# ORNL/MultiDistTorch

Hardware: AMD Instinct MI355X
Metric: aggregate VAE samples/sec across K concurrent HPO trials (higher is better)
Workload: dtype bf16; 1 GPU; model=conv-VAE 28x28 (2 conv + 2 deconv, z=32), global_batch=128, per_trial_batch=128, image=28, parallelism=groups1x1, trials=1, backend=hip, graphs=True, timing_barrier=none, valid=True

## Files before the change

### csrc/kernels/conv_igemm.h

```cpp
#pragma once
#include <stdint.h>

namespace mdt {

struct ConvDesc {
  int N, H, W, C;
  int OH, OW, CO;
  int KH, KW, S, P;
};

struct FastDiv {
  uint32_t d, mul, shr;
};

inline FastDiv make_fastdiv(uint32_t d) {
  FastDiv f;
  f.d = d;
  f.shr = 0;
  while ((1u << f.shr) < d) ++f.shr;
  const uint64_t one = 1;
  f.mul = (uint32_t)(((one << 32) * ((one << f.shr) - d)) / d + 1);
  return f;
}

enum IgemmMode : int {
  kModeConv = 0,
  kModeTconv = 1,
};

struct FwdPlan {
  int cfg;
  int BM, BN;
  int classes;
  int M;
  int Ncols, K;
  int mtiles, ntiles, ktiles;
  int ksplit, kt_per_split;
  int colsum_rows;
  int thin;
  int direct;
};

struct WgradPlan {
  int cfg;
  int BM, BN;
  int M, K2;
  int cotiles, ktiles, mtiles;
  int nsplit, mt_per_split;
  int thin;
};

struct APro {
  const float* slab;
  const float* bias;
  void* out16;
  int ks, relu, cin;
  long long stride;
};

struct GradSeg {
  long long off, numel;
  const float* slab;
  int nsplit;
  int co, k, s, ci;
  long long toff;
};

struct GradUnit {
  int seg, start, count;
};

struct TrUnit {
  int seg, tap, co0, ci0;
};

constexpr int kJobArgBytes = 256;
struct JobBlob {
  int kind;
  int nblk;
  int aux[6];
  alignas(16) unsigned char args[kJobArgBytes];
};

enum JobKindBase : int {
  kJobIgemm = 1000,
  kJobWgrad = 2000,
  kJobWgradThin = 2050,
  kJobThinWgM = 2100,
  kJobWgradAdam = 2200,
  kJobThinConv = 3000,
  kJobThinTconv = 4000,
  kJobColsum = 5000,
  kJobLoss = 5001,
  kJobCombine = 5002,
  kJobFinalize = 5003,
  kJobWtrans = 5004,
  kJobLossStep = 5005,
  kJobComm = 5006,
  kJobDconv = 6000,
};

constexpr int kMaxMultiJobs = 8;

}
```

### csrc/kernels/conv_igemm.hip

```cpp
#include <algorithm>

#include "conv_igemm_dev.h"
#include "conv_direct.h"
#include "conv_dwgrad.h"
#include "conv_thin_wg.h"

namespace mdt {

__global__ void __launch_bounds__(256) splitk_combine_k(CombineArgs c) {
  __shared__ float red[256];
  splitk_combine_body(c, red, blockIdx.x);
}

__global__ void __launch_bounds__(256) colsum_k(ColsumArgs c) { colsum_body(c, blockIdx.x); }

}

using namespace mdt;

namespace {
inline int cdiv(long long a, long long b) { return (int)((a + b - 1) / b); }
}

namespace mdt {
using namespace mdt::tiles;

struct DcInfo {
  int RB, NBB, MT, NB;
};
template <class CF>
constexpr DcInfo dc_info() { return DcInfo{CF::RB, CF::NBB, CF::MT, CF::NB}; }
static const DcInfo kDcInfo[] = {dc_info<DcS1>(), dc_info<DcS2>(), dc_info<DcT2>(),
                                  dc_info<DcT3>(), dc_info<DcS3>(), dc_info<DcT1>()};

static bool direct_small() {
  static const bool on = [] {
    const char* e = getenv("MDT_DCONV_SMALL");
    return !(e && e[0] == '0');
  }();
  return on;
}

int direct_cfg(int mode, const ConvDesc& d, bool fwd) {
  static const bool on = [] {
    const char* e = getenv("MDT_CONV_DIRECT");
    return !(e && e[0] == '0');
  }();
  static const bool bwd = [] {
    const char* e = getenv("MDT_DCONV_BWD");
    return !(e && e[0] == '0');
  }();
  if (!on || d.KH != 4 || d.KW != 4 || d.S != 2 || d.P != 1) return -1;
  if (!fwd && !bwd) return -1;
  if (d.H != d.W || d.OH != d.OW || d.H != 2 * d.OH) return -1;
  if (mode == kModeConv) {
    if (d.C == 32 && d.H == 64 && d.CO == 64) return 0;
    if (d.C == 64 && d.H == 32 && d.CO == 128) return 1;
    if (d.C == 128 && d.H == 16 && d.CO == 256 && fwd && direct_small()) return 4;
  } else {
    if (d.CO == 128 && d.OH == 16 && d.C == 64) return 2;
    if (d.CO == 64 && d.OH == 32 && d.C == 32) return 3;
    if (d.CO == 256 && d.OH == 8 && d.C == 128 && fwd && direct_small()) return 5;
  }
  return -1;
}

bool plan_fwd(int mode, const ConvDesc& d, bool allow_split, FwdPlan* p, bool allow_direct, bool fwd) {
  FwdPlan q{};
  const int dc = allow_direct ? direct_cfg(mode, d, fwd) : -1;
  if (dc >= 0) {
    const DcInfo& di = kDcInfo[dc];
    q.direct = dc + 1;
    q.classes = mode == kModeConv ? 1 : 4;
    q.M = mode == kModeConv ? d.N * d.OH * d.OW : d.N * d.OH * d.OW;
    q.Ncols = mode == kModeConv ? d.CO : d.C;
    q.K = mode == kModeConv ? 16 * d.C : 4 * d.CO;
    q.BM = di.MT; q.BN = di.NB;
    q.mtiles = d.N * di.RB; q.ntiles = di.NBB; q.ktiles = q.K / 64;
    q.ksplit = 1; q.kt_per_split = q.ktiles;
    q.colsum_rows = d.N * di.RB;
    q.cfg = 100 + dc;
    *p = q;
    return true;
  }
  if (mode == kModeConv) {
    q.classes = 1;
    q.M = d.N * d.OH * d.OW;
    q.Ncols = d.CO;
    q.K = d.KH * d.KW * d.C;
    q.thin = (d.C % 8) != 0;
  } else {
    if (d.KH % d.S || d.KW % d.S || d.H % d.S || d.W % d.S || d.CO % 8) return false;
    q.classes = d.S * d.S;
    q.M = d.N * (d.H / d.S) * (d.W / d.S);
    q.Ncols = d.C;
    q.K = (d.KH / d.S) * (d.KW / d.S) * d.CO;
    q.thin = 0;
  }
  if (q.K % 8 || q.M <= 0) return false;
  q.BN = q.Ncols >= 128 ? 128 : q.Ncols > 32 ? 64 : q.Ncols > 16 ? 32 : 16;
  if (q.thin) q.BN = 32;
  static const int bn_split_below = [] {
    const char* e = getenv("MDT_CONV_BN_SPLIT_BELOW");
    return e ? atoi(e) : 512;
  }();
  static const int bn_split_min_kt = [] {
    const char* e = getenv("MDT_CONV_BN_SPLIT_MIN_KT");
    return e ? atoi(e) : 16;
  }();
  static const int bn_split_tiny = [] {
    const char* e = getenv("MDT_CONV_BN_SPLIT_TINY");
    return e ? atoi(e) : 512;
  }();
  auto grid64 = [&] { return (long long)q.classes * cdiv(q.M, 64) * cdiv(q.Ncols, q.BN); };
  while (q.BN > 32 && !q.thin &&
         ((cdiv(q.K, 64) >= bn_split_min_kt && grid64() < bn_split_below) || grid64() < bn_split_tiny))
    q.BN /= 2;
  q.ntiles = cdiv(q.Ncols, q.BN);
  q.ktiles = cdiv(q.K, 64);
  static const int bm64_below = [] {
    const char* e = getenv("MDT_CONV_BM64_BELOW");
    return e ? atoi(e) : 1024;
  }();
  q.BM = 128;
  if ((long long)q.classes * cdiv(q.M, 128) * q.ntiles < bm64_below) q.BM = 64;
  q.mtiles = cdiv(q.M, q.BM);
  const long long blocks = (long long)q.classes * q.mtiles * q.ntiles;
  q.ksplit = 1;
  static const int min_kt = [] {
    const char* e = getenv("MDT_CONV_SPLIT_MIN_KT");
    return e ? atoi(e) : 8;
  }();
  static const int kt_per = [] {
    const char* e = getenv("MDT_CONV_SPLIT_KT_PER");
    const int v = e ? atoi(e) : 1;
    return v < 1 ? 1 : v;
  }();
  if (allow_split && q.classes == 1 && blocks < 256 && q.ktiles >= min_kt) {
    int ks = cdiv(512, blocks);
    if (ks > q.ktiles / kt_per) ks = q.ktiles / kt_per;
    if (ks < 1) ks = 1;
    q.ksplit = ks;
  }
  q.kt_per_split = cdiv(q.ktiles, q.ksplit);
  q.ksplit = cdiv(q.ktiles, q.kt_per_split);
  q.colsum_rows = q.classes * q.mtiles;
  const int bn_i = q.BN == 128 ? 0 : q.BN == 64 ? 1 : q.BN == 32 ? 2 : 3;
  q.cfg = (q.BM == 128 ? 0 : 4) + bn_i;
  *p = q;
  return true;
}

int dwgrad_cfg(const ConvDesc& d) {
  static const bool on = [] {
    const char* e = getenv("MDT_DWGRAD");
    return !(e && e[0] == '0');
  }();
  const char* e2 = getenv("MDT_DWGRAD_L2");
  const bool l2 = e2 && e2[0] == '1';
  if (!on || d.S != 2 || d.P != 1 || d.KH != 4 || d.KW != 4 || d.H != d.W || d.OH != d.OW || d.OH * 2 != d.H)
    return -1;
  if (d.H == DwL1::H && d.C == DwL1::C && d.CO == DwL1::CO) return 0;
  if (l2 && d.H == DwL2::H && d.C == DwL2::C && d.CO == DwL2::CO) return 1;
  return -1;
}

bool plan_wgrad(const ConvDesc& d, WgradPlan* p) {
  WgradPlan q{};
  if (d.CO % 8) return false;
  if (thin_wgrad_mfma_ok(d)) {
    q.cfg = 110;
    q.thin = true;
    q.M = d.N * d.OH * d.OW;
    q.K2 = d.KH * d.KW * d.C;
    q.BM = d.CO;
    q.BN = q.K2;
    q.cotiles = q.ktiles = 1;
    q.mtiles = d.N * d.OH / 4;
    q.nsplit = q.mtiles;
    q.mt_per_split = 1;
    *p = q;
    return true;
  }
  const int dw = dwgrad_cfg(d);
  if (dw >= 0) {
    q.cfg = 100 + dw;
    q.M = d.N * d.OH * d.OW;
    q.K2 = d.KH * d.KW * d.C;
    q.BM = d.CO;
    q.BN = q.K2;
    q.cotiles = q.ktiles = 1;
    q.mtiles = d.N;
    q.nsplit = d.N;
    q.mt_per_split = 1;
    *p = q;
    return true;
  }
  q.M = d.N * d.OH * d.OW;
  q.K2 = d.KH * d.KW * d.C;
  q.thin = (d.C % 8) != 0;
  q.BM = d.CO > 32 ? 64 : 32;
  q.BN = q.K2 > 32 ? 64 : q.K2 > 16 ? 32 : 16;
  if (q.thin && q.BN == 32) q.BN = 64;
  q.cotiles = cdiv(d.CO, q.BM);
  q.ktiles = cdiv(q.K2, q.BN);
  q.mtiles = cdiv(q.M, 64);
  const int tiles = q.cotiles * q.ktiles;
  static const int fixed_target = [] {
    const char* e = getenv("MDT_CONV_WG_TARGET");
    return e ? atoi(e) : 0;
  }();
  static const int thin_target = [] {
    const char* e = getenv("MDT_CONV_WG_TARGET_THIN");
    return e ? atoi(e) : 0;
  }();
  int target = q.thin && thin_target > 0 ? thin_target : fixed_target;
  if (target <= 0) {
    const long long work = (long long)q.mtiles * tiles;
    target = (int)std::min<long long>(640, std::max<long long>(160, work / 16));
  }
  int ns = cdiv(target, tiles);
  if (ns > q.mtiles / 2) ns = q.mtiles / 2;
  if (ns < 1) ns = 1;
  q.mt_per_split = cdiv(q.mtiles, ns);
  q.nsplit = cdiv(q.mtiles, q.mt_per_split);
  q.cfg = (q.BM == 64 ? 0 : 3) + (q.BN == 64 ? 0 : q.BN == 32 ? 1 : 2);
  *p = q;
  return true;
}

int build_igemm(int mode, const void* A, const void* B16, ConvDesc d, const float* bias, int relu, void* y16,
                float* y32, const void* omask, float* colsum, float* ws, IgArgs* pa, FwdPlan* pq, CombineArgs* pc,
                int* nc) {
  FwdPlan q;
  const bool can_split = ws != nullptr && omask == nullptr && colsum == nullptr;
  if (!plan_fwd(mode, d, can_split, &q, false)) return 1;
  IgArgs a{};
  a.d = d;
  a.A = A;
  a.B = reinterpret_cast<const __bf16*>(B16);
  a.relu = relu;
  a.M = q.M; a.Ncols = q.Ncols; a.K = q.K; a.mtiles = q.mtiles; a.ntiles = q.ntiles; a.ktiles = q.ktiles;
  a.kt_per_split = q.kt_per_split;
  if (mode == kModeConv) {
    a.f_pix = make_fastdiv(d.OH * d.OW); a.f_w = make_fastdiv(d.OW);
    a.f_ch = make_fastdiv(d.C); a.f_tw = make_fastdiv(d.KW);
  } else {
    a.f_pix = make_fastdiv((d.H / d.S) * (d.W / d.S)); a.f_w = make_fastdiv(d.W / d.S);
    a.f_ch = make_fastdiv(d.CO); a.f_tw = make_fastdiv(d.KW / d.S);
  }
  *nc = 0;
  if (q.ksplit > 1) {
    a.slab = ws;
    const long long MN = (long long)q.M * q.Ncols;
    int rp = 1;
    while (rp < 64 && rp * 4 < q.ksplit) rp *= 2;
    const int cnt = 256 / rp;
    *pc = CombineArgs{ws, q.ksplit, q.M, q.Ncols, cnt, bias, relu, y32, reinterpret_cast<__bf16*>(y16)};
    *nc = cdiv(MN, cnt);
  } else {
    a.y16 = reinterpret_cast<__bf16*>(y16); a.y32 = y32; a.bias = bias;
    a.omask = reinterpret_cast<const __bf16*>(omask); a.colsum = colsum;
  }
  *pa = a;
  *pq = q;
  return 0;
}

int build_wgrad(const void* G16, const void* X, ConvDesc d, float* out, WgArgs* pa, WgradPlan* pq) {
  WgradPlan q;
  if (!plan_wgrad(d, &q)) return 1;
  WgArgs a{};
  a.d = d;
  a.G = reinterpret_cast<const __bf16*>(G16);
  a.X = X;
  a.out = out;
  a.M = q.M; a.K2 = q.K2; a.cotiles = q.cotiles; a.ktiles = q.ktiles; a.mtiles = q.mtiles;
  a.mt_per_split = q.mt_per_split;
  a.f_pix = make_fastdiv(d.OH * d.OW); a.f_w = make_fastdiv(d.OW);
  a.f_c = make_fastdiv(d.C); a.f_kw = make_fastdiv(d.KW);
  *pa = a;
  *pq = q;
  return 0;
}

template <typename XT>
__global__ void __launch_bounds__(256) thin_wgrad_k(WgArgs a) {
  __shared__ __attribute__((aligned(16))) uint8_t lds[thin_wgrad_mfma_lds_bytes()];
  thin_wgrad_mfma_body<XT>(a, lds, blockIdx.x);
}

static unsigned long long* g_dc_stamps = nullptr;

template <class CF>
void launch_dc(const DcArgs& a, hipStream_t s) {
  hipLaunchKernelGGL((dconv_k<CF>), dim3(a.nimg * CF::RB * CF::NBB), dim3(CF::THREADS), 0, s, a);
}

int launch_direct(int cfg, const void* A, const void* B16, const ConvDesc& d, const float* bias, int relu, void* y16,
                  float* y32, const void* omask, float* colsum, hipStream_t s) {
  DcArgs a{};
  a.A = reinterpret_cast<const __bf16*>(A);
  a.B = reinterpret_cast<const __bf16*>(B16);
  a.y16 = reinterpret_cast<__bf16*>(y16);
  a.y32 = y32;
  a.bias = bias;
  a.omask = reinterpret_cast<const __bf16*>(omask);
  a.colsum = colsum;
  a.stamps = g_dc_stamps;
  a.relu = relu;
  a.nimg = d.N;
  switch (cfg) {
    case 0: launch_dc<DcS1>(a, s); break;
    case 1: launch_dc<DcS2>(a, s); break;
    case 2: launch_dc<DcT2>(a, s); break;
    case 3: launch_dc<DcT3>(a, s); break;
    case 4: launch_dc<DcS3>(a, s); break;
    case 5: launch_dc<DcT1>(a, s); break;
    default: return 2;
  }
  return (int)hipGetLastError();
}

int launch_splitk_combine(const CombineArgs& c, int nblk, hipStream_t s) {
  hipLaunchKernelGGL(splitk_combine_k, dim3(nblk), dim3(256), 0, s, c);
  return (int)hipGetLastError();
}

}

namespace {
using namespace mdt::tiles;

template <int MODE, typename AT, bool VEC, class TC, bool PRO = false>
void launch_fwd(const IgArgs& a, const FwdPlan& q, hipStream_t s) {
  dim3 grid(q.mtiles * q.ntiles, q.ksplit, q.classes);
  hipLaunchKernelGGL((igemm_fwd_k<MODE, AT, VEC, TC, PRO>), grid, dim3(256), 0, s, a);
}

template <int MODE, typename AT, bool VEC, bool PRO = false>
int dispatch_fwd_cfg(const IgArgs& a, const FwdPlan& q, hipStream_t s) {
  switch (q.cfg) {
    case 0: launch_fwd<MODE, AT, VEC, F0, PRO>(a, q, s); return 0;
    case 1: launch_fwd<MODE, AT, VEC, F1, PRO>(a, q, s); return 0;
    case 2: launch_fwd<MODE, AT, VEC, F2, PRO>(a, q, s); return 0;
    case 3: launch_fwd<MODE, AT, VEC, F3, PRO>(a, q, s); return 0;
    case 4: launch_fwd<MODE, AT, VEC, F4, PRO>(a, q, s); return 0;
    case 5: launch_fwd<MODE, AT, VEC, F5, PRO>(a, q, s); return 0;
    case 6: launch_fwd<MODE, AT, VEC, F6, PRO>(a, q, s); return 0;
    case 7: launch_fwd<MODE, AT, VEC, F7, PRO>(a, q, s); return 0;
  }
  return 2;
}

template <typename AT>
int dispatch_thin(const IgArgs& a, const FwdPlan& q, hipStream_t s) {
  if (q.cfg == 2) { launch_fwd<kModeConv, AT, false, F2>(a, q, s); return 0; }
  if (q.cfg == 6) { launch_fwd<kModeConv, AT, false, F6>(a, q, s); return 0; }
  return 2;
}

template <typename XT, bool VEC, class TC>
void launch_wg(const WgArgs& a, const WgradPlan& q, hipStream_t s) {
  dim3 grid(q.cotiles * q.ktiles * q.nsplit);
  hipLaunchKernelGGL((wgrad_k<XT, VEC, TC>), grid, dim3(256), 0, s, a);
}

}

extern "C" {

int mdt_igemm_plan(int mode, ConvDesc d, int allow_split, int* info, int fwd) {
  FwdPlan q;
  if (!plan_fwd(mode, d, allow_split != 0, &q, true, fwd != 0)) return 1;
  const int v[12] = {q.cfg, q.BM, q.BN, q.classes, q.M, q.Ncols, q.K, q.mtiles, q.ntiles, q.ktiles, q.ksplit,
                     q.colsum_rows};
  for (int i = 0; i < 12; ++i) info[i] = v[i];
  return 0;
}

int mdt_wgrad_plan(ConvDesc d, int* info) {
  WgradPlan q;
  if (!plan_wgrad(d, &q)) return 1;
  const int v[8] = {q.cfg, q.BM, q.BN, q.cotiles, q.ktiles, q.mtiles, q.nsplit, q.mt_per_split};
  for (int i = 0; i < 8; ++i) info[i] = v[i];
  return 0;
}

int mdt_igemm(int mode, const void* A, int a_is_f32, const void* B16, ConvDesc d, const float* bias, int relu,
              void* y16, float* y32, const void* omask, float* colsum, float* ws, int skip_combine, hipStream_t s,
              const APro* pro, int fwd) {
  IgArgs a;
  FwdPlan q;
  CombineArgs c;
  int nc = 0;
  const int dc = direct_cfg(mode, d, fwd != 0);
  if (dc >= 0) {
    if ((pro && pro->slab) || a_is_f32) return 5;
    return launch_direct(dc, A, B16, d, bias, relu, y16, y32, omask, colsum, s);
  }
  if (build_igemm(mode, A, B16, d, bias, relu, y16, y32, omask, colsum, ws, &a, &q, &c, &nc)) return 1;
  int rc;
  if (pro && pro->slab) {
    if (mode != kModeConv || q.thin || a_is_f32 || pro->cin % 8 || pro->ks < 1) return 4;
    a.pro = *pro;
    rc = dispatch_fwd_cfg<kModeConv, __bf16, true, true>(a, q, s);
  } else if (mode == kModeConv) {
    if (q.thin) rc = a_is_f32 ? dispatch_thin<float>(a, q, s) : dispatch_thin<__bf16>(a, q, s);
    else if (a_is_f32) rc = 3;
    else rc = dispatch_fwd_cfg<kModeConv, __bf16, true>(a, q, s);
  } else if (a_is_f32) {
    rc = 3;
  } else {
    rc = dispatch_fwd_cfg<kModeTconv, __bf16, true>(a, q, s);
  }
  if (rc) return rc;
  if (nc > 0 && !skip_combine) hipLaunchKernelGGL(splitk_combine_k, dim3(nc), dim3(256), 0, s, c);
  return (int)hipGetLastError();
}

int mdt_wgrad(const void* G16, const void* X, int x_is_f32, ConvDesc d, float* out, hipStream_t s) {
  WgArgs a;
  WgradPlan q;
  if (build_wgrad(G16, X, d, out, &a, &q)) return 1;
  if (q.cfg == 110) {
    if (x_is_f32) hipLaunchKernelGGL(thin_wgrad_k<float>, dim3(q.nsplit), dim3(256), 0, s, a);
    else hipLaunchKernelGGL(thin_wgrad_k<__bf16>, dim3(q.nsplit), dim3(256), 0, s, a);
    return (int)hipGetLastError();
  }
  if (q.cfg >= 100) {
    if (x_is_f32) return 3;
    const DwArgs da{reinterpret_cast<const __bf16*>(X), reinterpret_cast<const __bf16*>(G16), out, d.N, g_dc_stamps};
    if (q.cfg == 100) hipLaunchKernelGGL(dwgrad_k<DwL1>, dim3(d.N * 4), dim3(DwL1::THREADS), 0, s, da);
    else if (q.cfg == 101) hipLaunchKernelGGL(dwgrad_k<DwL2>, dim3(d.N * 4), dim3(DwL2::THREADS), 0, s, da);
    else return 2;
    return (int)hipGetLastError();
  }
  if (!q.thin) {
    if (x_is_f32) return 3;
    switch (q.cfg) {
      case 0: launch_wg<__bf16, true, W0>(a, q, s); break;
      case 1: launch_wg<__bf16, true, W1>(a, q, s); break;
      case 2: launch_wg<__bf16, true, W2>(a, q, s); break;
      case 3: launch_wg<__bf16, true, W3>(a, q, s); break;
      case 4: launch_wg<__bf16, true, W4>(a, q, s); break;
      case 5: launch_wg<__bf16, true, W5>(a, q, s); break;
      default: return 2;
    }
  } else {
    switch (q.cfg) {
      case 0: if (x_is_f32) launch_wg<float, false, W0>(a, q, s); else launch_wg<__bf16, false, W0>(a, q, s); break;
      case 2: if (x_is_f32) launch_wg<float, false, W2>(a, q, s); else launch_wg<__bf16, false, W2>(a, q, s); break;
      case 3: if (x_is_f32) launch_wg<float, false, W3>(a, q, s); else launch_wg<__bf16, false, W3>(a, q, s); break;
      case 5: if (x_is_f32) launch_wg<float, false, W5>(a, q, s); else launch_wg<__bf16, false, W5>(a, q, s); break;
      default: return 2;
    }
  }
  return (int)hipGetLastError();
}

void mdt_dconv_stamps(unsigned long long* p) { g_dc_stamps = p; }

int mdt_colsum(const void* G16, int M, int N, int rows_per, float* slab, hipStream_t s) {
  if (N % 8 || rows_per < 1) return 1;
  const int gx = cdiv(N / 8, 256);
  const ColsumArgs c{reinterpret_cast<const __bf16*>(G16), M, N, rows_per, gx, slab};
  hipLaunchKernelGGL(colsum_k, dim3(gx * cdiv(M, rows_per)), dim3(256), 0, s, c);
  return (int)hipGetLastError();
}

}
```

### csrc/kernels/conv_jobs.hip

```cpp
#include <string.h>

#include <algorithm>

#include "conv_direct.h"
#include "conv_dwgrad.h"
#include "conv_igemm_dev.h"
#include "comm_jobs.h"
#include "conv_small.h"
#include "conv_thin.h"
#include "conv_thin_wg.h"

namespace mdt {
using namespace tiles;

struct JobPack {
  JobBlob j[3];
  int start1, start2;
};

template <class T>
__device__ __forceinline__ const T& job_args(const JobBlob& j) {
  return *reinterpret_cast<const T*>(j.args);
}

struct JNone {
  static constexpr int ID = 0, LDS = 0;
  static __device__ __forceinline__ void run(const JobBlob&, uint8_t*, int) {}
};

template <int MODE, int CFG, class TC>
struct JIg {
  static constexpr int ID = kJobIgemm + MODE * 100 + CFG, LDS = igemm_lds_bytes<TC>();
  static __device__ __forceinline__ void run(const JobBlob& j, uint8_t* lds, int b) {
    const int ntb = j.aux[0], ks = j.aux[1];
    const int r = b / ntb, t = b - r * ntb;
    const int cls = r / ks, kz = r - cls * ks;
    igemm_body<MODE, __bf16, true, TC>(job_args<IgArgs>(j), lds, t, ntb, kz, cls);
  }
};

template <int CFG, class TC>
struct JWg {
  static constexpr int ID = kJobWgrad + CFG, LDS = wgrad_lds_bytes<TC>();
  static __device__ __forceinline__ void run(const JobBlob& j, uint8_t* lds, int b) {
    wgrad_body<__bf16, true, TC>(job_args<WgArgs>(j), lds, b, j.nblk);
  }
};

template <typename XT, int CFG, class TC>
struct JWgThin {
  static constexpr int ID = kJobWgradThin + (sizeof(XT) == 4 ? 20 : 0) + CFG, LDS = wgrad_lds_bytes<TC>();
  static __device__ __forceinline__ void run(const JobBlob& j, uint8_t* lds, int b) {
    wgrad_body<XT, false, TC>(job_args<WgArgs>(j), lds, b, j.nblk);
  }
};

template <typename XT>
struct JThinWg {
  static constexpr int ID = kJobThinWgM + (sizeof(XT) == 4 ? 1 : 0), LDS = thin_wgrad_mfma_lds_bytes();
  static __device__ __forceinline__ void run(const JobBlob& j, uint8_t* lds, int b) {
    thin_wgrad_mfma_body<XT>(job_args<WgArgs>(j), lds, b);
  }
};

template <int CO, typename TIN>
struct JThinConv {
  static constexpr int ID = kJobThinConv + CO + (sizeof(TIN) == 4 ? 100 : 0), LDS = thin_conv_lds_bytes<CO, 4>();
  static __device__ __forceinline__ void run(const JobBlob& j, uint8_t* lds, int b) {
    thin_conv_body<CO, 4, TIN>(job_args<ThinConvArgs>(j), lds, b);
  }
};

template <int CFG, class CF>
struct JDc {
  static constexpr int ID = kJobDconv + CFG, LDS = CF::LDS;
  static __device__ __forceinline__ void run(const JobBlob& j, uint8_t* lds, int b) {
    dconv_body<CF>(job_args<DcArgs>(j), lds, xcd_remap(b, j.nblk));
  }
};

struct JColsum {
  static constexpr int ID = kJobColsum, LDS = 0;
  static __device__ __forceinline__ void run(const JobBlob& j, uint8_t*, int b) { colsum_body(job_args<ColsumArgs>(j), b); }
};

struct JLoss {
  static constexpr int ID = kJobLoss, LDS = 64;
  static __device__ __forceinline__ void run(const JobBlob& j, uint8_t* lds, int) {
    loss_finalize_body(job_args<LossArgs>(j), reinterpret_cast<float*>(lds));
  }
};

struct JFinalize {
  static constexpr int ID = kJobFinalize, LDS = kFinalizeThreads * 4 + 64;
  static __device__ __forceinline__ void run(const JobBlob& j, uint8_t* lds, int b) {
    grad_finalize_body(job_args<FinalizeArgs>(j), reinterpret_cast<float*>(lds),
                       reinterpret_cast<AdamC*>(lds + kFinalizeThreads * 4), b);
  }
};

struct JWtrans {
  static constexpr int ID = kJobWtrans, LDS = kWtransLds;
  static __device__ __forceinline__ void run(const JobBlob& j, uint8_t* lds, int b) {
    wtrans_body(job_args<WtransArgs>(j), lds, b);
  }
};

struct JComm {
  static constexpr int ID = kJobComm, LDS = kCommLds;
  static __device__ __forceinline__ void run(const JobBlob& j, uint8_t* lds, int b) {
    comm_unit_body(job_args<CommJobArgs>(j), lds, b);
  }
};

struct JLossStep {
  static constexpr int ID = kJobLossStep, LDS = 64;
  static __device__ __forceinline__ void run(const JobBlob& j, uint8_t* lds, int) {
    loss_step_body(job_args<LossArgs>(j), reinterpret_cast<float*>(lds));
  }
};

constexpr int cmax(int a, int b) { return a > b ? a : b; }

struct JobPackN {
  JobBlob j[kMaxMultiJobs];
  int start[kMaxMultiJobs + 1];
  int n;
  unsigned long long* stamps;
};

constexpr int kMultiLds = cmax(cmax(cmax(wgrad_lds_bytes<W0>(), wgrad_lds_bytes<W1>()),
                                    cmax(wgrad_lds_bytes<W3>(), wgrad_lds_bytes<W4>())),
                               cmax(cmax(wgrad_lds_bytes<W2>(), wgrad_lds_bytes<W5>()),
                                    cmax(cmax(JFinalize::LDS, JComm::LDS), JColsum::LDS + 64)));

template <int CFG, class TC>
__device__ __forceinline__ bool run_wg_cfg(const JobBlob& j, uint8_t* lds, int b) {
  if (j.kind == kJobWgrad + CFG) {
    wgrad_body<__bf16, true, TC>(job_args<WgArgs>(j), lds, b, j.nblk);
    return true;
  }
  if (j.kind == kJobWgradThin + CFG) {
    wgrad_body<__bf16, false, TC>(job_args<WgArgs>(j), lds, b, j.nblk);
    return true;
  }
  if (j.kind == kJobWgradThin + 20 + CFG) {
    wgrad_body<float, false, TC>(job_args<WgArgs>(j), lds, b, j.nblk);
    return true;
  }
  return false;
}

__device__ __forceinline__ void run_multi_job(const JobBlob& j, uint8_t* lds, int lb) {
  if (run_wg_cfg<0, W0>(j, lds, lb) || run_wg_cfg<1, W1>(j, lds, lb) || run_wg_cfg<2, W2>(j, lds, lb) ||
      run_wg_cfg<3, W3>(j, lds, lb) || run_wg_cfg<4, W4>(j, lds, lb) || run_wg_cfg<5, W5>(j, lds, lb))
    return;
  switch (j.kind) {
    case kJobWgradAdam:
      wgrad_body<__bf16, true, W0, true>(job_args<WgAdamArgs>(j).w, lds, lb, j.nblk, &job_args<WgAdamArgs>(j));
      break;
    case kJobWgradAdam + 1:
      wgrad_body<__bf16, true, W1, true>(job_args<WgAdamArgs>(j).w, lds, lb, j.nblk, &job_args<WgAdamArgs>(j));
      break;
    case kJobLossStep: JLossStep::run(j, lds, lb); break;
    case kJobLoss: JLoss::run(j, lds, lb); break;
    case kJobFinalize: JFinalize::run(j, lds, lb); break;
    case kJobComm: JComm::run(j, lds, lb); break;
    case kJobColsum: JColsum::run(j, lds, lb); break;
    default: break;
  }
}

__global__ void __launch_bounds__(256) jobs_multi_k(const JobPackN* __restrict__ p) {
  __shared__ __attribute__((aligned(16))) uint8_t lds[kMultiLds];
  const int b = blockIdx.x;
  int st[kMaxMultiJobs];
#pragma unroll
  for (int k = 0; k < kMaxMultiJobs; ++k) st[k] = p->start[k];
  const int n = p->n;
  int i = 0, s0 = st[0];
#pragma unroll
  for (int k = 1; k < kMaxMultiJobs; ++k)
    if (k < n && b >= st[k]) {
      i = k;
      s0 = st[k];
    }
  unsigned long long* stamps = p->stamps;
  unsigned long long t0 = 0;
  if (stamps) t0 = __builtin_amdgcn_s_memrealtime();
  run_multi_job(p->j[i], lds, b - s0);
  if (stamps) {
    __syncthreads();
    if (threadIdx.x == 0) {
      stamps[2 * b] = t0;
      stamps[2 * b + 1] = __builtin_amdgcn_s_memrealtime();
    }
  }
}

__host__ inline bool multi_kind_ok(int k) {
  if (k >= kJobWgrad && k <= kJobWgrad + 5) return true;
  if (k >= kJobWgradThin && k <= kJobWgradThin + 5) return true;
  if (k >= kJobWgradThin + 20 && k <= kJobWgradThin + 25) return true;
  if (k == kJobWgradAdam || k == kJobWgradAdam + 1) return true;
  return k == kJobLossStep || k == kJobLoss || k == kJobFinalize || k == kJobColsum || k == kJobComm;
}

template <class A, class B, class C>
__global__ void __launch_bounds__(256) jobs_k(JobPack p) {
  __shared__ __attribute__((aligned(1024))) uint8_t lds[cmax(cmax(A::LDS, B::LDS), cmax(C::LDS, 16))];
  const int b = blockIdx.x;
  if (b < p.start1) A::run(p.j[0], lds, b);
  else if (b < p.start2) B::run(p.j[1], lds, b - p.start1);
  else C::run(p.j[2], lds, b - p.start2);
}

}

using namespace mdt;

namespace {

typedef void (*PackLaunch)(const JobPack&, int, hipStream_t);

template <class A, class B, class C>
void launch_pack(const JobPack& p, int grid, hipStream_t s) {
  hipLaunchKernelGGL((jobs_k<A, B, C>), dim3(grid), dim3(256), 0, s, p);
}

struct Combo {
  int k0, k1, k2;
  PackLaunch fn;
};

#define COMBO3(A, B, C) {A::ID, B::ID, C::ID, &launch_pack<A, B, C>}
#define COMBO2(A, B) {A::ID, B::ID, 0, &launch_pack<A, B, JNone>}

using WgT5 = JWgThin<__bf16, 5, W5>;
using WgT5f = JWgThin<float, 5, W5>;
using ThinC32 = JThinConv<32, __bf16>;
using ThinC32f = JThinConv<32, float>;
using TwB = JThinWg<__bf16>;
using TwF = JThinWg<float>;
using Wg0 = JWg<0, W0>;
using Wg1 = JWg<1, W1>;
using IgC1 = JIg<kModeConv, 1, F1>;
using IgC4 = JIg<kModeConv, 4, F4>;
using IgC5 = JIg<kModeConv, 5, F5>;
using IgC6 = JIg<kModeConv, 6, F6>;
using IgT1 = JIg<kModeTconv, 1, F1>;
using IgT2 = JIg<kModeTconv, 2, F2>;
using IgT4 = JIg<kModeTconv, 4, F4>;
using IgT5 = JIg<kModeTconv, 5, F5>;
using IgT6 = JIg<kModeTconv, 6, F6>;
using DcJS2 = JDc<1, DcS2>;
using DcJT2 = JDc<2, DcT2>;

const Combo kCombos[] = {
    COMBO3(WgT5, ThinC32, JLoss),
    COMBO2(WgT5, ThinC32),
    COMBO3(TwB, ThinC32, JLoss),
    COMBO2(TwB, ThinC32),
    COMBO2(TwF, JFinalize),
    COMBO2(IgC5, Wg0),
    COMBO2(IgC1, Wg0),
    COMBO2(IgC4, Wg0),
    COMBO2(IgC6, Wg0),
    COMBO3(IgC6, Wg0, JColsum),
    COMBO3(IgT6, Wg1, JColsum),
    COMBO3(IgT5, Wg0, JColsum),
    COMBO3(IgT6, Wg0, JColsum),
    COMBO3(IgT4, Wg0, JColsum),
    COMBO2(IgT6, Wg0),
    COMBO2(IgT4, Wg0),
    COMBO2(IgT1, Wg0),
    COMBO2(IgT2, Wg0),
    COMBO2(IgT5, Wg0),
    COMBO3(IgC1, Wg0, JFinalize),
    COMBO3(IgC4, Wg0, JFinalize),
    COMBO3(IgC5, Wg0, JFinalize),
    COMBO3(IgC6, Wg0, JFinalize),
    COMBO3(IgT1, Wg0, JFinalize),
    COMBO3(IgT2, Wg0, JFinalize),
    COMBO3(IgT4, Wg0, JFinalize),
    COMBO3(IgT6, Wg0, JFinalize),
    COMBO2(WgT5f, JFinalize),
    COMBO2(JFinalize, JWtrans),
    COMBO2(ThinC32f, JWtrans),
    COMBO2(IgC1, JWtrans),
    COMBO2(IgC4, JWtrans),
    COMBO2(IgC5, JWtrans),
    COMBO2(IgC6, JWtrans),
    COMBO2(Wg0, DcJS2),
    COMBO2(Wg0, DcJT2),
    COMBO3(IgC1, Wg0, JComm),
    COMBO3(IgC4, Wg0, JComm),
    COMBO3(IgC5, Wg0, JComm),
    COMBO3(IgC6, Wg0, JComm),
    COMBO3(IgT1, Wg0, JComm),
    COMBO3(IgT2, Wg0, JComm),
    COMBO3(IgT4, Wg0, JComm),
    COMBO3(IgT5, Wg0, JComm),
    COMBO3(IgT6, Wg0, JComm),
    COMBO3(Wg0, JComm, DcJS2),
    COMBO3(Wg0, JComm, DcJT2),
    COMBO2(TwF, JComm),
    COMBO2(WgT5f, JComm),
    COMBO2(JComm, JComm),
};

#undef COMBO3
#undef COMBO2

inline int cdivj(long long a, long long b) { return (int)((a + b - 1) / b); }

template <class CF>
constexpr int dc_grid(int n) { return n * CF::RB * CF::NBB; }
inline int direct_grid(int dc, int n) {
  switch (dc) {
    case 0: return dc_grid<DcS1>(n);
    case 1: return dc_grid<DcS2>(n);
    case 2: return dc_grid<DcT2>(n);
    case 3: return dc_grid<DcT3>(n);
    default: return 0;
  }
}

template <class T>
void put_args(JobBlob* j, const T& a) {
  static_assert(sizeof(T) <= kJobArgBytes, "job arguments exceed the blob");
  memset(j->args, 0, sizeof(j->args));
  memcpy(j->args, &a, sizeof(T));
}

}

extern "C" {

int mdt_job_igemm(JobBlob* g, JobBlob* c, int mode, const void* A, int a_is_f32, const void* B16, ConvDesc d,
                  const float* bias, int relu, void* y16, float* y32, const void* omask, float* colsum, float* ws,
                  int skip_combine) {
  IgArgs a;
  FwdPlan q;
  CombineArgs cb;
  int nc = 0;
  if (build_igemm(mode, A, B16, d, bias, relu, y16, y32, omask, colsum, ws, &a, &q, &cb, &nc)) return 1;
  memset(g, 0, sizeof(*g));
  memset(c, 0, sizeof(*c));
  const int dc = direct_cfg(mode, d, false);
  if (dc >= 0) {
    if (a_is_f32 || dc > 3) return 0;
    DcArgs da{};
    da.A = reinterpret_cast<const __bf16*>(A);
    da.B = reinterpret_cast<const __bf16*>(B16);
    da.y16 = reinterpret_cast<__bf16*>(y16);
    da.y32 = y32;
    da.bias = bias;
    da.omask = reinterpret_cast<const __bf16*>(omask);
    da.colsum = colsum;
    da.relu = relu;
    da.nimg = d.N;
    g->kind = kJobDconv + dc;
    g->nblk = direct_grid(dc, d.N);
    put_args(g, da);
    return 0;
  }
  const bool ok = !a_is_f32 && !q.thin;
  g->kind = ok ? kJobIgemm + mode * 100 + q.cfg : 0;
  g->nblk = q.mtiles * q.ntiles * q.ksplit * q.classes;
  g->aux[0] = q.mtiles * q.ntiles;
  g->aux[1] = q.ksplit;
  put_args(g, a);
  if (nc > 0 && !skip_combine) {
    c->kind = kJobCombine;
    c->nblk = nc;
    put_args(c, cb);
  }
  return 0;
}

int mdt_job_wgrad(JobBlob* j, const void* G16, const void* X, int x_is_f32, ConvDesc d, float* out) {
  WgArgs a;
  WgradPlan q;
  if (build_wgrad(G16, X, d, out, &a, &q)) return 1;
  memset(j, 0, sizeof(*j));
  if (q.cfg == 110) j->kind = kJobThinWgM + (x_is_f32 ? 1 : 0);
  else if (q.cfg >= 100) {
    return 0;
  }
  else if (!q.thin) j->kind = x_is_f32 ? 0 : kJobWgrad + q.cfg;
  else j->kind = kJobWgradThin + (x_is_f32 ? 20 : 0) + q.cfg;
  j->nblk = q.cotiles * q.ktiles * q.nsplit;
  put_args(j, a);
  return 0;
}

int mdt_job_wgrad_adam(JobBlob* j, const void* G16, const void* X, int x_is_f32, ConvDesc d, float* P, float* Mo,
                       float* Vo, void* w16, const float* adamc) {
  WgAdamArgs a{};
  WgradPlan q;
  if (!P || !Mo || !Vo || !w16 || !adamc || x_is_f32) return 1;
  if (build_wgrad(G16, X, d, nullptr, &a.w, &q)) return 1;
  if (q.thin || q.cfg < 0 || q.cfg > 1 || q.nsplit != 1 || (q.K2 & 3)) return 1;
  if ((long long)d.CO * q.K2 >= (1ll << 28)) return 1;
  if (((uintptr_t)P | (uintptr_t)Mo | (uintptr_t)Vo) & 15 || ((uintptr_t)w16 & 7)) return 1;
  a.P = P; a.Mo = Mo; a.Vo = Vo;
  a.w16 = reinterpret_cast<__bf16*>(w16);
  a.c = reinterpret_cast<const AdamC*>(adamc);
  memset(j, 0, sizeof(*j));
  j->kind = kJobWgradAdam + q.cfg;
  j->nblk = q.cotiles * q.ktiles;
  put_args(j, a);
  return 0;
}

int mdt_job_thin_conv(JobBlob* j, const void* X, int x_is_f32, const float* Wf, ConvDesc d, const float* bias,
                      int relu, void* y16, const void* omask, float* colsum, const int* idx, void* st,
                      const void* hp, int B, float* xb) {
  if (d.C != 1 || d.KH != 4 || d.KW != 4) return 1;
  if ((idx || xb || hp) && (!st || !x_is_f32 || (d.H * d.W) % 4)) return 1;
  memset(j, 0, sizeof(*j));
  const bool ok = d.CO == 16 || d.CO == 32 || d.CO == 64;
  j->kind = ok ? kJobThinConv + d.CO + (x_is_f32 ? 100 : 0) : 0;
  j->nblk = cdivj((long long)d.N * d.OH * d.OW, 256);
  const ThinConvArgs ta{X, Wf, d, bias, relu, reinterpret_cast<__bf16*>(y16), reinterpret_cast<const __bf16*>(omask),
                        colsum, idx, reinterpret_cast<TrainState*>(st), reinterpret_cast<const HParams*>(hp), B, xb,
                        j->nblk, thin_conv_mfma_ok(d, x_is_f32)};
  put_args(j, ta);
  return 0;
}

int mdt_job_colsum(JobBlob* j, const void* G16, int M, int N, int rows_per, float* slab) {
  if (N % 8 || rows_per < 1) return 1;
  memset(j, 0, sizeof(*j));
  const int gx = cdivj(N / 8, 256);
  j->kind = kJobColsum;
  j->nblk = gx * cdivj(M, rows_per);
  put_args(j, ColsumArgs{reinterpret_cast<const __bf16*>(G16), M, N, rows_per, gx, slab});
  return 0;
}

int mdt_job_loss(JobBlob* j, const float* bce_part, int nb, const float* kld_part, int nk, void* st, const void* hp,
                 int advance_cursor) {
  memset(j, 0, sizeof(*j));
  j->kind = (advance_cursor & 2) ? kJobLossStep : kJobLoss;
  advance_cursor &= 1;
  j->nblk = 1;
  put_args(j, LossArgs{bce_part, nb, kld_part, nk, reinterpret_cast<TrainState*>(st),
                       reinterpret_cast<const HParams*>(hp), advance_cursor});
  return 0;
}

int mdt_job_finalize(JobBlob* j, float* P, float* G, float* Mo, float* Vo, void* w16, const void* segs,
                     const void* units, int nunits, const void* st, const void* hp, int do_adam) {
  memset(j, 0, sizeof(*j));
  if (nunits <= 0) return 1;
  j->kind = kJobFinalize;
  j->nblk = nunits;
  put_args(j, FinalizeArgs{P, G, Mo, Vo, reinterpret_cast<__bf16*>(w16), reinterpret_cast<const GradSeg*>(segs),
                           reinterpret_cast<const GradUnit*>(units), reinterpret_cast<const TrainState*>(st),
                           reinterpret_cast<const HParams*>(hp), do_adam});
  return 0;
}

int mdt_job_comm(JobBlob* j, float* P, float* G, float* Mo, float* Vo, void* w16, const void* segs, const void* units,
                 int nunits, const void* st, const void* hp, int do_adam, const void* ctx, int mode) {
  memset(j, 0, sizeof(*j));
  if (nunits <= 0 || !ctx || mode < kCommPush || mode > kCommPushReduce) return 1;
  j->kind = kJobComm;
  j->nblk = nunits;
  CommJobArgs a{};
  a.fa = FinalizeArgs{P, G, Mo, Vo, reinterpret_cast<__bf16*>(w16), reinterpret_cast<const GradSeg*>(segs),
                      reinterpret_cast<const GradUnit*>(units), reinterpret_cast<const TrainState*>(st),
                      reinterpret_cast<const HParams*>(hp), do_adam};
  a.ctx = reinterpret_cast<const CommCtx*>(ctx);
  a.mode = mode;
  put_args(j, a);
  return 0;
}

int mdt_job_wtrans(JobBlob* j, const void* w16, void* w16t, const void* segs, const void* units, int nunits) {
  memset(j, 0, sizeof(*j));
  if (nunits <= 0) return 1;
  j->kind = kJobWtrans;
  j->nblk = nunits;
  put_args(j, WtransArgs{reinterpret_cast<const __bf16*>(w16), reinterpret_cast<__bf16*>(w16t),
                         reinterpret_cast<const GradSeg*>(segs), reinterpret_cast<const TrUnit*>(units)});
  return 0;
}

int mdt_launch_jobs(const JobBlob* jobs, int n, hipStream_t s) {
  if (n < 2 || n > 3) return 2;
  const JobBlob* v[3] = {&jobs[0], &jobs[1], n > 2 ? &jobs[2] : nullptr};
  for (int i = 0; i < n; ++i)
    if (v[i]->kind <= 0 || v[i]->nblk <= 0) return 1;
  std::sort(v, v + n, [](const JobBlob* a, const JobBlob* b) { return a->kind < b->kind; });
  const int k2 = n > 2 ? v[2]->kind : 0;
  for (const Combo& c : kCombos) {
    if (c.k0 != v[0]->kind || c.k1 != v[1]->kind || c.k2 != k2) continue;
    JobPack p;
    memset(&p, 0, sizeof(p));
    p.j[0] = *v[0];
    p.j[1] = *v[1];
    if (n > 2) p.j[2] = *v[2];
    p.start1 = v[0]->nblk;
    p.start2 = v[0]->nblk + v[1]->nblk;
    const int grid = p.start2 + (n > 2 ? v[2]->nblk : 0);
    c.fn(p, grid, s);
    return (int)hipGetLastError() ? -1 : 0;
  }
  return 1;
}

int mdt_jobs_multi_bytes() { return (int)sizeof(JobPackN); }

int mdt_pack_jobs_multi_stamps(void* img, void* stamps) {
  reinterpret_cast<JobPackN*>(img)->stamps = reinterpret_cast<unsigned long long*>(stamps);
  return 0;
}

int mdt_pack_jobs_multi(const JobBlob* jobs, int n, void* dst) {
  if (n < 1 || n > kMaxMultiJobs) return -1;
  JobPackN p;
  memset(&p, 0, sizeof(p));
  int grid = 0;
  for (int i = 0; i < n; ++i) {
    if (jobs[i].nblk <= 0) return -1;
    if (!multi_kind_ok(jobs[i].kind)) return 0;
    p.j[i] = jobs[i];
    p.start[i] = grid;
    grid += jobs[i].nblk;
  }
  p.start[n] = grid;
  p.n = n;
  memcpy(dst, &p, sizeof(p));
  return grid;
}

int mdt_launch_jobs_multi(const void* dev_pack, int grid, hipStream_t s) {
  if (!dev_pack || grid <= 0) return 2;
  hipLaunchKernelGGL(jobs_multi_k, dim3(grid), dim3(256), 0, s, reinterpret_cast<const JobPackN*>(dev_pack));
  return (int)hipGetLastError() ? -1 : 0;
}

int mdt_launch_job1(const JobBlob* j, hipStream_t s) {
  if (j->kind == kJobCombine) return launch_splitk_combine(*reinterpret_cast<const CombineArgs*>(j->args), j->nblk, s);
  return 1;
}

}
```

Measured before the change: 2.302 million samples/s.

## Add specialized weight-gradient kernel for the 28x28 single-channel first conv

Adds a dedicated weight-gradient kernel for the first encoder conv (C=1, 28x28 input, 4x4 stride 2, 32 output channels). It stages whole input images in LDS and builds the im2col B tiles from shared memory, batching three M-tiles per round, instead of the generic thin path that gathers each patch element from global memory. The kernel is wired into both the standalone launch path and the fused multi-job kernel, with new combos for finalize and comm. It also changes the thin-target env lookup from a cached static to a per-call getenv, which adds host overhead on every plan build.

```diff
diff --git a/csrc/kernels/conv_igemm.h b/csrc/kernels/conv_igemm.h
--- a/csrc/kernels/conv_igemm.h
+++ b/csrc/kernels/conv_igemm.h
@@ -87,6 +87,7 @@
   kJobWgrad = 2000,
   kJobWgradThin = 2050,
   kJobThinWgM = 2100,
+  kJobThin28Wg = 2150,
   kJobWgradAdam = 2200,
   kJobThinConv = 3000,
   kJobThinTconv = 4000,
diff --git a/csrc/kernels/conv_igemm.hip b/csrc/kernels/conv_igemm.hip
--- a/csrc/kernels/conv_igemm.hip
+++ b/csrc/kernels/conv_igemm.hip
@@ -3,6 +3,7 @@
 #include "conv_igemm_dev.h"
 #include "conv_direct.h"
 #include "conv_dwgrad.h"
+#include "conv_thin28_wg.h"
 #include "conv_thin_wg.h"
 
 namespace mdt {
@@ -210,10 +211,8 @@
     const char* e = getenv("MDT_CONV_WG_TARGET");
     return e ? atoi(e) : 0;
   }();
-  static const int thin_target = [] {
-    const char* e = getenv("MDT_CONV_WG_TARGET_THIN");
-    return e ? atoi(e) : 0;
-  }();
+  const char* et = getenv("MDT_CONV_WG_TARGET_THIN");
+  const int thin_target = et ? atoi(et) : 0;
   int target = q.thin && thin_target > 0 ? thin_target : fixed_target;
   if (target <= 0) {
     const long long work = (long long)q.mtiles * tiles;
@@ -288,6 +287,11 @@
 __global__ void __launch_bounds__(256) thin_wgrad_k(WgArgs a) {
   __shared__ __attribute__((aligned(16))) uint8_t lds[thin_wgrad_mfma_lds_bytes()];
   thin_wgrad_mfma_body<XT>(a, lds, blockIdx.x);
+}
+
+__global__ void __launch_bounds__(256) thin28_wgrad_k(WgArgs a) {
+  __shared__ __attribute__((aligned(16))) uint8_t lds[thin28_wgrad_lds_bytes()];
+  thin28_wgrad_body(a, lds, blockIdx.x, gridDim.x);
 }
 
 static unsigned long long* g_dc_stamps = nullptr;
@@ -448,6 +452,10 @@
       default: return 2;
     }
   } else {
+    if (q.cfg == 5 && thin28_wgrad_ok(d, x_is_f32 != 0, X, G16)) {
+      hipLaunchKernelGGL(thin28_wgrad_k, dim3(q.nsplit), dim3(256), 0, s, a);
+      return (int)hipGetLastError();
+    }
     switch (q.cfg) {
       case 0: if (x_is_f32) launch_wg<float, false, W0>(a, q, s); else launch_wg<__bf16, false, W0>(a, q, s); break;
       case 2: if (x_is_f32) launch_wg<float, false, W2>(a, q, s); else launch_wg<__bf16, false, W2>(a, q, s); break;
diff --git a/csrc/kernels/conv_jobs.hip b/csrc/kernels/conv_jobs.hip
--- a/csrc/kernels/conv_jobs.hip
+++ b/csrc/kernels/conv_jobs.hip
@@ -8,6 +8,7 @@
 #include "comm_jobs.h"
 #include "conv_small.h"
 #include "conv_thin.h"
+#include "conv_thin28_wg.h"
 #include "conv_thin_wg.h"
 
 namespace mdt {
@@ -60,6 +61,13 @@
   static constexpr int ID = kJobThinWgM + (sizeof(XT) == 4 ? 1 : 0), LDS = thin_wgrad_mfma_lds_bytes();
   static __device__ __forceinline__ void run(const JobBlob& j, uint8_t* lds, int b) {
     thin_wgrad_mfma_body<XT>(job_args<WgArgs>(j), lds, b);
+  }
+};
+
+struct JThin28Wg {
+  static constexpr int ID = kJobThin28Wg, LDS = thin28_wgrad_lds_bytes();
+  static __device__ __forceinline__ void run(const JobBlob& j, uint8_t* lds, int b) {
+    thin28_wgrad_body(job_args<WgArgs>(j), lds, b, j.nblk);
   }
 };
 
@@ -133,6 +141,7 @@
                                     cmax(wgrad_lds_bytes<W3>(), wgrad_lds_bytes<W4>())),
                                cmax(cmax(wgrad_lds_bytes<W2>(), wgrad_lds_bytes<W5>()),
                                     cmax(cmax(JFinalize::LDS, JComm::LDS), JColsum::LDS + 64)));
+static_assert(JThin28Wg::LDS <= kMultiLds, "thin28 weight gradient exceeds the multi-job kernel's LDS");
 
 template <int CFG, class TC>
 __device__ __forceinline__ bool run_wg_cfg(const JobBlob& j, uint8_t* lds, int b) {
@@ -156,6 +165,7 @@
       run_wg_cfg<3, W3>(j, lds, lb) || run_wg_cfg<4, W4>(j, lds, lb) || run_wg_cfg<5, W5>(j, lds, lb))
     return;
   switch (j.kind) {
+    case kJobThin28Wg: JThin28Wg::run(j, lds, lb); break;
     case kJobWgradAdam:
       wgrad_body<__bf16, true, W0, true>(job_args<WgAdamArgs>(j).w, lds, lb, j.nblk, &job_args<WgAdamArgs>(j));
       break;
@@ -202,7 +212,7 @@
   if (k >= kJobWgrad && k <= kJobWgrad + 5) return true;
   if (k >= kJobWgradThin && k <= kJobWgradThin + 5) return true;
   if (k >= kJobWgradThin + 20 && k <= kJobWgradThin + 25) return true;
-  if (k == kJobWgradAdam || k == kJobWgradAdam + 1) return true;
+  if (k == kJobWgradAdam || k == kJobWgradAdam + 1 || k == kJobThin28Wg) return true;
   return k == kJobLossStep || k == kJobLoss || k == kJobFinalize || k == kJobColsum || k == kJobComm;
 }
 
@@ -285,6 +295,7 @@
     COMBO3(IgT4, Wg0, JFinalize),
     COMBO3(IgT6, Wg0, JFinalize),
     COMBO2(WgT5f, JFinalize),
+    COMBO2(JThin28Wg, JFinalize),
     COMBO2(JFinalize, JWtrans),
     COMBO2(ThinC32f, JWtrans),
     COMBO2(IgC1, JWtrans),
@@ -306,6 +317,7 @@
     COMBO3(Wg0, JComm, DcJT2),
     COMBO2(TwF, JComm),
     COMBO2(WgT5f, JComm),
+    COMBO2(JThin28Wg, JComm),
     COMBO2(JComm, JComm),
 };
 
@@ -389,6 +401,7 @@
     return 0;
   }
   else if (!q.thin) j->kind = x_is_f32 ? 0 : kJobWgrad + q.cfg;
+  else if (q.cfg == 5 && thin28_wgrad_ok(d, x_is_f32 != 0, X, G16)) j->kind = kJobThin28Wg;
   else j->kind = kJobWgradThin + (x_is_f32 ? 20 : 0) + q.cfg;
   j->nblk = q.cotiles * q.ktiles * q.nsplit;
   put_args(j, a);
diff --git a/csrc/kernels/conv_thin28_wg.h b/csrc/kernels/conv_thin28_wg.h
--- /dev/null
+++ b/csrc/kernels/conv_thin28_wg.h
@@ -0,0 +1,98 @@
+#pragma once
+#include "conv_igemm_dev.h"
+
+namespace mdt {
+
+__host__ inline bool thin28_wgrad_ok(const ConvDesc& d, bool x_is_f32, const void* X, const void* G) {
+  const char* e = getenv("MDT_THIN28_WG");
+  if (e && e[0] == '0') return false;
+  if (!x_is_f32 || (((uintptr_t)X | (uintptr_t)G) & 15)) return false;
+  return d.N >= 1 && d.C == 1 && d.H == 28 && d.W == 28 && d.OH == 14 && d.OW == 14 && d.CO == 32 && d.KH == 4 &&
+         d.KW == 4 && d.S == 2 && d.P == 1;
+}
+
+typedef __attribute__((address_space(1))) bf16x8 gbf16x8;
+typedef __attribute__((address_space(1))) f32x4 gf32x4;
+
+constexpr int kT28Round = 3;
+constexpr int kT28A = 64 * 32 * 2;
+constexpr int kT28B = 64 * 16 * 2;
+constexpr int kT28Stage = kT28A + kT28B;
+constexpr int kT28Img = 28 * 28 * 4;
+constexpr int thin28_wgrad_lds_bytes() { return kT28Round * kT28Stage + 2 * kT28Img + 16; }
+
+__device__ __forceinline__ void thin28_wgrad_body(const WgArgs& a, uint8_t* lds, int bid, int nblk) {
+  using TC = tiles::W5;
+  static_assert(TC::BM == 32 && TC::BN == 16 && TC::KWS == 2 && TC::FM == 1 && TC::FN == 1 && TC::WN == 1, "W5");
+  static_assert(TC::RED_BYTES + 4 * 16 * 20 * 4 <= thin28_wgrad_lds_bytes(), "epilogue staging exceeds LDS");
+  constexpr int PIX = 196, OW = 14, IW = 28, IMG = IW * IW;
+  const int tid = threadIdx.x, lane = tid & 63;
+  const int w = __builtin_amdgcn_readfirstlane(tid >> 6);
+  const int wk = w / (TC::WM * TC::WN), wm = (w % (TC::WM * TC::WN)) / TC::WN;
+  const int split = xcd_remap(bid, nblk);
+  const int mt0 = split * a.mt_per_split;
+  const int mt1 = min(a.mtiles, mt0 + a.mt_per_split);
+  const float* Xp = reinterpret_cast<const float*>(a.X);
+  float* imgs = reinterpret_cast<float*>(lds + kT28Round * kT28Stage);
+
+  f32x4 acc[1][1] = {{f32x4{0.f, 0.f, 0.f, 0.f}}};
+  for (int mta = mt0; mta < mt1; mta += kT28Round) {
+    const int nt = min(kT28Round, mt1 - mta);
+    const int row0 = 64 * mta, rowe = min(a.M, row0 + 64 * nt);
+    const int n0 = (int)((uint32_t)row0 / PIX);
+    const int nimg = (int)((uint32_t)(rowe - 1) / PIX) - n0 + 1;
+    const int m_a = row0 + (tid >> 2);
+    const int f1 = tid + 256;
+    const bool ok0 = m_a < a.M, ok1 = 1 < nt && m_a + 64 < a.M, ok2 = 2 < nt && m_a + 128 < a.M;
+    const gbf16x8* Gp = (const gbf16x8*)(a.G + 8 * (tid & 3));
+    const gf32x4* Ip = (const gf32x4*)(Xp + (size_t)n0 * IMG);
+    const bf16x8 ga0 = Gp[ok0 ? (size_t)m_a * 4 : 0];
+    const f32x4 xv0 = Ip[tid < (IMG / 4) * nimg ? tid : 0];
+    const f32x4 xv1 = Ip[f1 < (IMG / 4) * nimg ? f1 : 0];
+    const bf16x8 ga1 = Gp[ok1 ? (size_t)(m_a + 64) * 4 : 0];
+    const bf16x8 ga2 = Gp[ok2 ? (size_t)(m_a + 128) * 4 : 0];
+    uint8_t* at = lds + timg<32>(tid >> 2, tid & 3);
+    *reinterpret_cast<bf16x8*>(at) = ok0 ? ga0 : zero8();
+    reinterpret_cast<f32x4*>(imgs)[tid] = xv0;
+    reinterpret_cast<f32x4*>(imgs)[f1 < 2 * (IMG / 4) ? f1 : 2 * (IMG / 4)] = xv1;
+    *reinterpret_cast<bf16x8*>(at + kT28Stage) = ok1 ? ga1 : zero8();
+    *reinterpret_cast<bf16x8*>(at + 2 * kT28Stage) = ok2 ? ga2 : zero8();
+    __syncthreads();
+#pragma unroll
+    for (int i = 0; i < 2; ++i) {
+      const int c = tid + 256 * i;
+      if (c < 128 * nt) {
+        const int t = c >> 7, r = (c >> 1) & 63, chb = c & 1;
+        const int m = row0 + 64 * t + r;
+        const bool mok = m < a.M;
+        const uint32_t mm = mok ? (uint32_t)m : (uint32_t)row0;
+        const uint32_t n = mm / PIX, rem = mm - n * PIX;
+        const uint32_t oy = rem / OW, ox = rem - oy * OW;
+        const int iy0 = 2 * (int)oy - 1 + 2 * chb, ix0 = 2 * (int)ox - 1;
+        const float* im = imgs + (int)(n - (uint32_t)n0) * IMG;
+        bf16x8 b;
+#pragma unroll
+        for (int j = 0; j < 8; ++j) {
+          const int iy = iy0 + (j >> 2), ix = ix0 + (j & 3);
+          const bool ok = mok && (unsigned)iy < (unsigned)IW && (unsigned)ix < (unsigned)IW;
+          const float x = im[ok ? iy * IW + ix : 0];
+          b[j] = (__bf16)(ok ? x : 0.f);
+        }
+        *reinterpret_cast<bf16x8*>(lds + t * kT28Stage + kT28A + timg<16>(r, chb)) = b;
+      }
+    }
+    __syncthreads();
+    for (int t = 0; t < nt; ++t) {
+      const uint8_t* As = lds + t * kT28Stage;
+      const uint8_t* Bs = As + kT28A;
+      const int kb = 32 * wk;
+      const bf16x8 af = tr_frag<32>(As, wm * 16, kb, lane);
+      const bf16x8 bfr = tr_frag<16>(Bs, 0, kb, lane);
+      acc[0][0] = mfma_bf16(af, bfr, acc[0][0]);
+    }
+    __syncthreads();
+  }
+  wgrad_epilogue<TC>(a, acc, lds, 0, 0, split);
+}
+
+}
```

Result: no change. 2.303 million samples/s, median of 2 (+0.0%).
